# CEA-LIST/runia_core

Hardware: AMD Instinct MI355X
Metric: OOD scores/sec, LaREM 16-MC PCA-256 (ResNet-18 layer4 latent 512x4x4) (higher is better)
Workload: dtype f64

## Files before the change

### runia_core_amd/csrc/fused.hip

```cpp
#include "common.hpp"
#include "entropy_core.hpp"
#include "mfma_f64_tile.hpp"
#include "philox.hpp"
#include "div_consts.hpp"
#include "trap_order.hpp"

namespace {

using namespace runia_entropy;
using namespace runia_mfma;

constexpr int kMaxMC = 64;
typedef float f2 __attribute__((ext_vector_type(2)));

__device__ __forceinline__ void layer_consts(int cnt, int& m, float& flag, float& zh, float& zl) {
  const int a = cnt ? __ffs(cnt) - 1 : 0;
  m = cnt >> a;
  flag = __uint_as_float((unsigned)(127 - a) << 23);
  zh = cnt ? __uint_as_float(runia_div::kDivHi[(m - 1) >> 1]) : NAN;
  zl = cnt ? __uint_as_float(runia_div::kDivLo[(m - 1) >> 1]) : 0.f;
}

__device__ __forceinline__ float add_f32(float a, float b) {
  float r;
// ... 402 lines not shown
  const double* packed_ct;
  const double* bias;
  const double* scale;
  const double* md_mean;
  const double* packed_p;
  double* score;
  double* y_out;
  int64_t N, D, n;
};

template <int RT>
__global__ __launch_bounds__(256) void pca_md_kernel(PcaMdArgs g) {
  constexpr int BM = 16 * RT;
  extern __shared__ double lds[];
  const int64_t n_pad = n_padded(g.n);
  const int ypitch = (int)n_pad + 2;
  double* lds_a = lds;
  double* lds_y = lds + 2 * BM * APITCH;
  double* part = lds_y + (size_t)BM * ypitch;
  const int tid = threadIdx.x, lane = tid & 63;
  const int wave = __builtin_amdgcn_readfirstlane(tid >> 6);
  const int li = lane & 15, lg = lane >> 4;
  const int64_t NT = n_pad / 16;
  const int64_t r0 = (int64_t)blockIdx.x * BM;

  if (g.packed_ct) {
    const int64_t nchunks = k_padded(g.D) / KC;
    constexpr int PER_T = BM * KC / 256;
    for (int64_t cb = 0; cb < n_pad / BN; ++cb) {
      const int64_t ctbase = cb * 16 + wave * 4;
      d4 acc[RT][4];
#pragma unroll
      for (int a = 0; a < RT; ++a)
#pragma unroll
        for (int c = 0; c < 4; ++c) acc[a][c] = (d4){0.0, 0.0, 0.0, 0.0};
      const double2* bp = reinterpret_cast<const double2*>(g.packed_ct) + ctbase * 64 + lane;
      double2 b0[4];
#pragma unroll
      for (int c = 0; c < 4; ++c) b0[c] = bp[c * 64];
      double areg[PER_T];
      const int srow = (tid * PER_T) / KC, skk = (tid * PER_T) % KC;
      auto load_a = [&](int64_t kc) {
        const int64_t gr = r0 + srow;
#pragma unroll
        for (int q = 0; q < PER_T; ++q) {
          const int64_t gk = kc + skk + q;
          areg[q] = (gr < g.N && gk < g.D) ? g.h[gr * g.D + gk] : 0.0;
        }
      };
      load_a(0);
      int buf = 0;
      for (int64_t ch = 0; ch < nchunks; ++ch) {
#pragma unroll
        for (int q = 0; q < PER_T; ++q) lds_a[(buf * BM + srow) * APITCH + skk + q] = areg[q];
        __syncthreads();
        if (ch + 1 < nchunks) load_a((ch + 1) * KC);
        mfma_chunk<RT>(acc, lds_a + buf * BM * APITCH, APITCH, li, lg, bp + ch * 4 * NT * 64, NT * 64, b0);
        buf ^= 1;
      }
#pragma unroll
      for (int a = 0; a < RT; ++a)
#pragma unroll
        for (int c = 0; c < 4; ++c) {
          const int64_t col = (ctbase + c) * 16 + li;
#pragma unroll
          for (int r = 0; r < 4; ++r) {
            const int row = 16 * a + lg + 4 * r;
            double d = 0.0;
            if (col < g.n) {
              double y = acc[a][c][r] - g.bias[col];
              if (g.scale) y = y / g.scale[col];
              if (g.y_out && r0 + row < g.N) g.y_out[(r0 + row) * g.n + col] = y;
              d = y - g.md_mean[col];
            }
            lds_y[row * ypitch + col] = d;
          }
        }
      __syncthreads();
    }
  } else {
    for (int i = tid; i < BM * (int)n_pad; i += 256) {
      const int row = i / (int)n_pad, col = i - row * (int)n_pad;
      double d = 0.0;
      if (r0 + row < g.N && col < g.n) d = g.h[(r0 + row) * g.D + col] - g.md_mean[col];
      lds_y[row * ypitch + col] = d;
    }
    __syncthreads();
  }

  double rowdot[RT][4];
#pragma unroll
  for (int a = 0; a < RT; ++a)
#pragma unroll
    for (int r = 0; r < 4; ++r) rowdot[a][r] = 0.0;
  const int64_t kchunks = k_padded(g.n) / KC;
  for (int64_t cb = 0; cb < n_pad / BN; ++cb) {
    const int64_t ctbase = cb * 16 + wave * 4;
    d4 acc[RT][4];
#pragma unroll
    for (int a = 0; a < RT; ++a)
#pragma unroll
      for (int c = 0; c < 4; ++c) acc[a][c] = (d4){0.0, 0.0, 0.0, 0.0};
    const double2* bp = reinterpret_cast<const double2*>(g.packed_p) + ctbase * 64 + lane;
    double2 b0[4];
#pragma unroll
    for (int c = 0; c < 4; ++c) b0[c] = bp[c * 64];
    for (int64_t ch = 0; ch < kchunks; ++ch)
      mfma_chunk<RT>(acc, lds_y + ch * KC, ypitch, li, lg, bp + ch * 4 * NT * 64, NT * 64, b0);
#pragma unroll
    for (int a = 0; a < RT; ++a)
#pragma unroll
      for (int c = 0; c < 4; ++c) {
        const int col = (int)((ctbase + c) * 16) + li;
#pragma unroll
        for (int r = 0; r < 4; ++r) rowdot[a][r] += acc[a][c][r] * lds_y[(16 * a + lg + 4 * r) * ypitch + col];
      }
  }
#pragma unroll
  for (int a = 0; a < RT; ++a)
#pragma unroll
    for (int r = 0; r < 4; ++r) {
      double v = rowdot[a][r];
      v += shfl_xor_f64(v, 1);
      v += shfl_xor_f64(v, 2);
      v += shfl_xor_f64(v, 4);
      v += shfl_xor_f64(v, 8);
      if (li == 0) part[wave * BM + 16 * a + lg + 4 * r] = v;
    }
  __syncthreads();
  if (tid < BM) {
    const int64_t row = r0 + tid;
    if (row < g.N) g.score[row] = -(((part[tid] + part[BM + tid]) + part[2 * BM + tid]) + part[3 * BM + tid]);
  }
}

struct ProjSqArgs {
  const double* h;
  const double* packed_m;
  const double* c;
  double* score;
  double* partial;
  int64_t N, D, r;
};

#ifndef K2_WAVES
#define K2_WAVES 5
#endif
#ifndef K2_DMA
#define K2_DMA 1
#endif
#ifndef K2_WAVES_DMA
#define K2_WAVES_DMA 5
#endif
#ifndef K2_TRAP_FORM
#define K2_TRAP_FORM 2
#endif
#ifndef K2_TRAP_ROT
#define K2_TRAP_ROT 2
#endif
#ifndef K2_TRAP_HALFMAP
#define K2_TRAP_HALFMAP 1
#endif
template <int RT, int NCT, bool ACCUMULATE, bool SPLIT, bool DMA, int TRAP = 0>
__global__ __launch_bounds__(256, (RT == 1 && NCT <= 2) ? (DMA ? K2_WAVES_DMA : K2_WAVES) : 1) void proj_sq_kernel(ProjSqArgs g) {
#if defined(__HIP_DEVICE_COMPILE__)
  constexpr int BM = 16 * RT;
  constexpr bool WAVE_SKIP = TRAP >= 2 && DMA && RT == 1;
  __shared__ double lds_a[DMA ? 1 : 2 * BM * APITCH];
  __shared__ __attribute__((aligned(16))) double lds_d0[DMA ? BM * KC : 2];
  __shared__ __attribute__((aligned(16))) double lds_d1[DMA ? BM * KC : 2];
  constexpr int NG = (NCT + 1) / 2;
  __shared__ double part[4 * NG * BM];
  const int64_t n_pad = n_padded(g.r);
  const int tid = threadIdx.x, lane = tid & 63;
  const int wave = __builtin_amdgcn_readfirstlane(tid >> 6);
  const int li = lane & 15, lg = lane >> 4;
  const int64_t NT = n_pad / 16;
  int64_t tile = blockIdx.x;
  int half = 0;
  if constexpr (SPLIT) {
    tile = (int64_t)(blockIdx.x >> 4) * 8 + (blockIdx.x & 7);
    const unsigned j = blockIdx.x >> 3;
    half = (int)((K2_TRAP_HALFMAP ? j ^ (j >> 5) : j) & 1);
    if (tile * BM >= g.N) return;
  }
  const int64_t r0 = tile * BM;
  const int nchunks = (int)(k_padded(g.D) / KC);
  const int rot = K2_TRAP_ROT == 1 ? (int)(tile & 3)
                  : K2_TRAP_ROT == 2 ? (int)(((blockIdx.x >> 4) + (blockIdx.x >> 8)) & 3)
                  : K2_TRAP_ROT == 3 ? (int)((blockIdx.x >> 8) & 3) : 0;
  const int grp = WAVE_SKIP ? (wave + rot) & 3 : wave;
  constexpr int PER_T = BM * KC / 256;
  double rowsq[NG][RT][4];
#pragma unroll
  for (int q = 0; q < NG; ++q)
#pragma unroll
    for (int a = 0; a < RT; ++a)
#pragma unroll
      for (int r = 0; r < 4; ++r) rowsq[q][a][r] = 0.0;
  for (int64_t cb = 0; cb < n_pad / BN; ++cb) {
    const int64_t ctbase = cb * 16 + (int64_t)half * (4 * NCT) + grp * NCT;
    int64_t wg_chunk = (cb * 16 + (int64_t)half * (4 * NCT)) * 16 / KC, wave_chunk = ctbase * 16 / KC;
    if constexpr (TRAP == 3) {
      const int64_t wg_pos = (cb * 16 + (int64_t)half * (4 * NCT)) / 2, wave_pos = ctbase / 2;
      wg_chunk = trap_balanced_first_k(wg_pos, g.r) / KC;
#pragma unroll
      for (int i = 1; i < 2 * NCT; ++i) {
        const int64_t f = trap_balanced_first_k(wg_pos + i, g.r) / KC;
        wg_chunk = f < wg_chunk ? f : wg_chunk;
      }
      wave_chunk = trap_balanced_first_k(wave_pos, g.r) / KC;
#pragma unroll
      for (int q = 1; q < NG; ++q) {
        const int64_t f = trap_balanced_first_k(wave_pos + q, g.r) / KC;
        wave_chunk = f < wave_chunk ? f : wave_chunk;
      }
    }
    const int ch0 = TRAP ? (int)(wg_chunk < nchunks - 1 ? wg_chunk : nchunks - 1) : 0;
    [[maybe_unused]] const int ws = WAVE_SKIP ? (int)(wave_chunk < nchunks - 1 ? wave_chunk : nchunks - 1) : ch0;
    d4 acc[RT][NCT];
#pragma unroll
    for (int a = 0; a < RT; ++a)
#pragma unroll
      for (int c = 0; c < NCT; ++c) acc[a][c] = (d4){0.0, 0.0, 0.0, 0.0};
    double2 bring[4][NCT];
    if constexpr (DMA) {
      const __amdgpu_buffer_rsrc_t brsrc = buffer_of(g.packed_m, (unsigned)(packed_elems(g.D, g.r) * 8));
      const int64_t rows_here = (g.N - r0 < BM) ? g.N - r0 : BM;
      const __amdgpu_buffer_rsrc_t arsrc = buffer_of(g.h + r0 * g.D, (unsigned)(rows_here * g.D * 8));
      const unsigned lane_bytes = (unsigned)lane * 16u;
      const unsigned pair_stride_bytes = (unsigned)NT * 1024u;
      const unsigned ct_bytes = (unsigned)ctbase * 1024u;
      constexpr int NDMA = BM / 4 / 4;
      unsigned a_lane_bytes[NDMA];
#pragma unroll
      for (int i = 0; i < NDMA; ++i) {
        const int slot = 64 * (wave + 4 * i) + lane;
        a_lane_bytes[i] = (unsigned)(((slot % BM) * g.D + 2 * (slot / BM)) * 8);
      }
      auto dma_rows = [&](int bufc, int kc) {
#pragma unroll
        for (int i = 0; i < NDMA; ++i)
          __builtin_amdgcn_raw_ptr_buffer_load_lds(
              arsrc, (__attribute__((address_space(3))) void*)((bufc ? lds_d1 : lds_d0) + 128 * (wave + 4 * i)), 16,
              a_lane_bytes[i], (unsigned)kc * 8u, 0, 0);
        asm volatile("" ::: "memory");
      };
      auto body = [&](auto buf_tag, int ch) {
        constexpr int bufc = decltype(buf_tag)::value;
        asm volatile("s_waitcnt vmcnt(%0)" ::"n"(3 * NCT) : "memory");
        __syncthreads();
        dma_rows(bufc ^ 1, ((ch + 1 < nchunks) ? ch + 1 : ch) * KC);
        mfma_chunk_dma<RT, NCT, BM>(acc, bufc ? lds_d1 : lds_d0, li, lg, brsrc, lane_bytes,
                                    ct_bytes + (unsigned)ch * 4u * pair_stride_bytes, pair_stride_bytes, bring);
      };
      dma_rows(0, ch0 * KC);
      int ch = ch0;
      if constexpr (WAVE_SKIP) {
        for (; ch < ws; ++ch) {
          asm volatile("s_waitcnt vmcnt(0)" ::: "memory");
          __syncthreads();
          dma_rows((ch + 1 - ch0) & 1, (ch + 1) * KC);
        }
      }
#pragma unroll
      for (int j = 0; j < 3; ++j)
#pragma unroll
        for (int c = 0; c < NCT; ++c)
          bring[j][c] = __builtin_bit_cast(double2, __builtin_amdgcn_raw_buffer_load_b128(
                                                        brsrc, lane_bytes + c * 1024u,
                                                        ct_bytes + (unsigned)(4 * ch + j) * pair_stride_bytes, 0));
      if constexpr (WAVE_SKIP) {
        if ((ch - ch0) & 1) {
          body(std::integral_constant<int, 1>{}, ch);
          ++ch;
        }
      }
      for (; ch + 1 < nchunks; ch += 2) {
        body(std::integral_constant<int, 0>{}, ch);
        body(std::integral_constant<int, 1>{}, ch + 1);
      }
      if (ch < nchunks) body(std::integral_constant<int, 0>{}, ch);
    } else {
      const double2* bp = reinterpret_cast<const double2*>(g.packed_m) + ctbase * 64 + lane + (int64_t)ch0 * 4 * NT * 64;
    #pragma unroll
      for (int j = 0; j < 3; ++j)
  #pragma unroll
        for (int c = 0; c < NCT; ++c) bring[j][c] = bp[j * NT * 64 + c * 64];
      double areg[PER_T];
      const int srow = tid / KC, skk = tid % KC;
      const bool interior = (r0 + BM <= g.N) && (g.D % KC == 0);
      const double* pa = g.h + (r0 + srow) * g.D + skk;
      auto load_a = [&](int64_t kc) {
        if (interior) {
  #pragma unroll
          for (int q = 0; q < PER_T; ++q) areg[q] = pa[(int64_t)q * (256 / KC) * g.D + kc];
          return;
        }
        const int64_t gk = kc + skk;
  #pragma unroll
        for (int q = 0; q < PER_T; ++q) {
          const int64_t gr = r0 + srow + q * (256 / KC);
          areg[q] = (gr < g.N && gk < g.D) ? g.h[gr * g.D + gk] : 0.0;
        }
      };
      load_a((int64_t)ch0 * KC);
      int buf = 0;
      for (int64_t ch = ch0; ch < nchunks; ++ch) {
  #pragma unroll
        for (int q = 0; q < PER_T; ++q) lds_a[(buf * BM + srow + q * (256 / KC)) * APITCH + skk] = areg[q];
        __syncthreads();
        if (ch + 1 < nchunks) load_a((ch + 1) * KC);
        mfma_chunk_ring<RT, NCT>(acc, lds_a + buf * BM * APITCH, APITCH, li, lg, bp + (ch - ch0) * 4 * NT * 64, NT * 64, bring);
        buf ^= 1;
      }
    }
#pragma unroll
    for (int a = 0; a < RT; ++a)
#pragma unroll
      for (int c = 0; c < NCT; ++c) {
        const int64_t col = (ctbase + c) * 16 + li;
        const double cc = (col < g.r) ? g.c[col] : 0.0;
#pragma unroll
        for (int r = 0; r < 4; ++r) {
          const double v = acc[a][c][r] + cc;
          rowsq[c / 2][a][r] = fma(v, v, rowsq[c / 2][a][r]);
        }
      }
    __syncthreads();
  }
#pragma unroll
  for (int q = 0; q < NG; ++q)
#pragma unroll
    for (int a = 0; a < RT; ++a)
#pragma unroll
      for (int r = 0; r < 4; ++r) {
        double v = rowsq[q][a][r];
        v += shfl_xor_f64(v, 1);
        v += shfl_xor_f64(v, 2);
        v += shfl_xor_f64(v, 4);
        v += shfl_xor_f64(v, 8);
        if (li == 0) part[(grp * NG + q) * BM + 16 * a + lg + 4 * r] = v;
      }
  __syncthreads();
  if (tid < BM) {
    const int64_t row = r0 + tid;
    if (row < g.N) {
      const double lo = ((part[tid] + part[BM + tid]) + part[2 * BM + tid]) + part[3 * BM + tid];
      if constexpr (NCT == 4) {
        const double hi = ((part[4 * BM + tid] + part[5 * BM + tid]) + part[6 * BM + tid]) + part[7 * BM + tid];
        g.score[row] = -(lo + hi);
      } else if constexpr (!SPLIT) {
        if constexpr (ACCUMULATE) unsafeAtomicAdd(&g.score[row], -lo);
        else g.score[row] = -lo;
      } else if constexpr (ACCUMULATE) {
        unsafeAtomicAdd(&g.score[row], -lo);
      } else {
        g.partial[(int64_t)half * g.N + row] = lo;
      }
    }
  }
#endif
}

__global__ void proj_sq_combine_kernel(const double* __restrict__ partial, double* __restrict__ score, int64_t N) {
  const int64_t i = (int64_t)blockIdx.x * blockDim.x + threadIdx.x;
  if (i < N) score[i] = -(partial[i] + partial[N + i]);
}

double digamma_diff(int n, int k) {
  double s = 0.0;
  for (int j = n - 1; j >= k; --j) s += 1.0 / (double)j;
  return s;
}

template <int RT>
int launch_pca_md(const PcaMdArgs& g, hipStream_t s) {
  constexpr int BM = 16 * RT;
  const int64_t n_pad = n_padded(g.n);
  const size_t shmem = ((size_t)2 * BM * APITCH + (size_t)BM * (n_pad + 2) + 4 * BM) * sizeof(double);
  if (shmem > 160 * 1024) return RUNIA_E_INVALID;
  static std::atomic<uint64_t> lds_ok{0};
  if (runia_allow_dynamic_lds(reinterpret_cast<const void*>(pca_md_kernel<RT>), 160 * 1024, lds_ok) != RUNIA_OK)
    return RUNIA_E_LAUNCH;
  const int64_t tiles = (g.N + BM - 1) / BM;
  pca_md_kernel<RT><<<(unsigned)tiles, 256, shmem, s>>>(g);
  return runia_check_launch();
}

}

extern "C" int runia_pca_md_score_f64(const double* h, const double* packed_ct, const double* bias,
                                      const double* scale, const double* md_mean, const double* packed_p,
                                      double* score, double* y_out, int64_t N, int64_t D, int64_t n,
                                      runia_stream_t stream) {
  if (N < 0 || D <= 0 || n <= 0) return RUNIA_E_INVALID;
  if (N == 0) return RUNIA_OK;
  if (!h || !md_mean || !packed_p || !score) return RUNIA_E_INVALID;
  if (packed_ct ? !bias : (n != D)) return RUNIA_E_INVALID;
  PcaMdArgs g{h, packed_ct, bias, scale, md_mean, packed_p, score, y_out, N, D, n};
  const int64_t tiles32 = (N + 31) / 32;
  const int64_t n_pad = n_padded(n);
  const bool fits32 = ((size_t)2 * 32 * APITCH + (size_t)32 * (n_pad + 2) + 128) * 8 <= 160 * 1024;
  if (tiles32 >= 1024 && fits32) return launch_pca_md<2>(g, as_stream(stream));
  return launch_pca_md<1>(g, as_stream(stream));
}

namespace {
template <int HH, int WW, int NPP>
void launch_mask(const float* rnd, int64_t rand_image_stride, float* table, int64_t N, int n_mc, float gamma,
                 int block_size, int identity, int sort_layers, uint64_t seed, int64_t first_image, int redraw,
                 hipStream_t s) {
  static_assert(HH * WW <= 64, "mc_mask_bits_kernel holds a drop layer in one 64-bit word");
  const unsigned grid = (unsigned)((N + kMaskBitsWaves - 1) / kMaskBitsWaves);
  if (redraw)
    mc_mask_bits_kernel<HH, WW, NPP, true><<<grid, 64 * kMaskBitsWaves, 0, s>>>(rnd, rand_image_stride, table, N, n_mc, gamma,
                                                                              block_size, identity, sort_layers, seed, first_image);
  else
    mc_mask_bits_kernel<HH, WW, NPP, false><<<grid, 64 * kMaskBitsWaves, 0, s>>>(rnd, rand_image_stride, table, N, n_mc, gamma,
                                                                               block_size, identity, sort_layers, seed, first_image);
}

__global__ void mc_draws_kernel(float* __restrict__ out, int64_t N, int per_image, uint64_t seed, int64_t first_image) {
  const int64_t i = (int64_t)blockIdx.x * blockDim.x + threadIdx.x;
  if (i >= N * per_image) return;
  const int64_t img = i / per_image;
  out[i] = runia_philox::draw(seed, (uint64_t)(first_image + img), (int)(i - img * per_image));
}
}

extern "C" int runia_mc_entropy_supported(int H, int W, int n_mc, int k);

extern "C" size_t runia_mc_entropy_workspace_bytes(int64_t N, int H, int W, int n_mc) {
  if (N <= 0 || H <= 0 || W <= 0 || n_mc <= 0) return 0;
  return (size_t)N * (size_t)n_mc * (size_t)(H * W + 2) * sizeof(float);
}

static int mc_args_ok(int64_t N, int H, int W, int n_mc, const void* workspace, size_t workspace_bytes) {
  if (N < 0 || N > 65535 || H <= 0 || W <= 0 || n_mc < 2 || n_mc > kMaxMC) return RUNIA_E_INVALID;
  if (N == 0) return RUNIA_OK;
  if (!workspace || workspace_bytes < runia_mc_entropy_workspace_bytes(N, H, W, n_mc) ||
      (((uintptr_t)workspace) & 15) != 0)
    return RUNIA_E_WORKSPACE;
  return RUNIA_OK;
}

#define RUNIA_MCE_SHAPES(F) \
  F(4, 4, 16, 5) F(4, 4, 32, 5) F(4, 4, 8, 5) F(2, 2, 16, 5) F(2, 2, 32, 5) F(7, 7, 16, 5) F(7, 7, 32, 5) F(8, 8, 16, 5) F(8, 8, 32, 5)

static int mc_mask_table(const float* rnd, int64_t rand_image_stride, void* workspace, size_t workspace_bytes,
                         int64_t N, int H, int W, int n_mc, double drop_prob, int block_size, int sort_layers,
                         runia_stream_t stream, bool counter = false, uint64_t seed = 0, int64_t first_image = 0,
                         int redraw = 0) {
  if (block_size < 1) return RUNIA_E_INVALID;
  if (int rc = mc_args_ok(N, H, W, n_mc, workspace, workspace_bytes)) return rc;
  if (N == 0) return RUNIA_OK;
  const int identity = (drop_prob == 0.0);
  if (!identity && !rnd && !counter) return RUNIA_E_INVALID;
  if (counter) rnd = nullptr;
  float* table = reinterpret_cast<float*>(workspace);
  const float gamma = (float)(drop_prob / (double)(block_size * block_size));
  hipStream_t s = as_stream(stream);
#define RUNIA_MCE(HH, WW, NPP, KK)                                                                          \
  if (H == HH && W == WW && n_mc <= NPP && n_mc > NPP / 2) {                                                \
    launch_mask<HH, WW, NPP>(rnd, rand_image_stride, table, N, n_mc, gamma, block_size, identity,           \
                             sort_layers, seed, first_image, redraw, s);                                    \
    return runia_check_launch();                                                                            \
  }
  RUNIA_MCE_SHAPES(RUNIA_MCE)
#undef RUNIA_MCE
  return RUNIA_E_INVALID;
}

extern "C" int runia_mc_mask_table_f32(const float* rnd, int64_t rand_image_stride, void* workspace,
                                       size_t workspace_bytes, int64_t N, int H, int W, int n_mc, double drop_prob,
                                       int block_size, runia_stream_t stream) {
  return mc_mask_table(rnd, rand_image_stride, workspace, workspace_bytes, N, H, W, n_mc, drop_prob, block_size, 1,
                       stream);
}

extern "C" int runia_mc_stack_table_f32(const float* x, const float* rnd, int64_t rand_image_stride, float* z,
                                        void* workspace, size_t workspace_bytes, int64_t N, int C, int H, int W,
                                        int n_mc, double drop_prob, int block_size, runia_stream_t stream) {
  if (C <= 0) return RUNIA_E_INVALID;
  if (int rc = mc_args_ok(N, H, W, n_mc, workspace, workspace_bytes)) return rc;
  if (N == 0) return RUNIA_OK;
  if (!x || !z || !runia_mc_entropy_supported(H, W, n_mc, 5)) return RUNIA_E_INVALID;
  if (!(((((uintptr_t)x) & 15) == 0) || (H * W) % 4 != 0)) return RUNIA_E_INVALID;
  if (int rc = mc_mask_table(rnd, rand_image_stride, workspace, workspace_bytes, N, H, W, n_mc, drop_prob,
                             block_size, 0, stream))
    return rc;
  const float* table = reinterpret_cast<const float*>(workspace);
  const unsigned grid = (unsigned)((((N + 7) / 8 + K1_IMGS - 1) / K1_IMGS) * 8 * ((C + kK1Block - 1) / kK1Block));
  hipStream_t s = as_stream(stream);
#define RUNIA_MCE(HH, WW, NPP, KK)                                                                          \
// ... 27 lines not shown
  const unsigned grid = (unsigned)((((N + 7) / 8 + K1_IMGS - 1) / K1_IMGS) * 8 * ((C + kK1Block - 1) / kK1Block));
  hipStream_t s = as_stream(stream);
  const bool x16 = ((((uintptr_t)x) & 15) == 0);
#define RUNIA_MCE(HH, WW, NPP, KK)                                                                          \
  if (H == HH && W == WW && n_mc <= NPP && n_mc > NPP / 2 && k == KK && (x16 || (HH * WW) % 4 != 0)) {      \
    if (n_mc == NPP)                                                                                        \
      RUNIA_LAUNCH_TIMED((mc_entropy_kernel<HH, WW, NPP, KK, true>), grid, kK1Block, 0, s, x, table, h, z_out, \
                         zero_fill, N, C, n_mc, min_dist, ct, inv_n);                                       \
    else                                                                                                    \
      RUNIA_LAUNCH_TIMED((mc_entropy_kernel<HH, WW, NPP, KK, false>), grid, kK1Block, 0, s, x, table, h, z_out, \
                         zero_fill, N, C, n_mc, min_dist, ct, inv_n);                                       \
    return runia_check_launch();                                                                            \
  }
  RUNIA_MCE_SHAPES(RUNIA_MCE)
#undef RUNIA_MCE
  return RUNIA_E_INVALID;
}

extern "C" int runia_mc_entropy_f32(const float* x, const float* rnd, int64_t rand_image_stride, double* h,
                                    float* z_out, double* zero_fill, void* workspace, size_t workspace_bytes,
                                    int64_t N, int C, int H, int W, int n_mc, double drop_prob, int block_size,
                                    int k, double min_dist, runia_stream_t stream) {
  if (N < 0 || C <= 0 || H <= 0 || W <= 0 || n_mc < 2 || n_mc > kMaxMC || block_size < 1 || k < 1 || k >= n_mc)
    return RUNIA_E_INVALID;
  if (N == 0) return RUNIA_OK;
  if (!x || !h || N > 65535) return RUNIA_E_INVALID;
  if (!runia_mc_entropy_supported(H, W, n_mc, k)) return RUNIA_E_INVALID;
  if (drop_prob != 0.0 && !rnd) return RUNIA_E_INVALID;
  if (!(((((uintptr_t)x) & 15) == 0) || (H * W) % 4 != 0)) return RUNIA_E_INVALID;
  if (int rc = runia_mc_mask_table_f32(rnd, rand_image_stride, workspace, workspace_bytes, N, H, W, n_mc, drop_prob,
                                       block_size, stream))
    return rc;
  return runia_mc_entropy_from_table_f32(x, workspace, workspace_bytes, h, z_out, zero_fill, N, C, H, W, n_mc, k,
                                         min_dist, stream);
}

int runia_roi_sample_table(const float* feat_nhwc, const float* boxes, const int* batch_idx, void* table, size_t table_bytes,
                           int64_t K, int64_t B, int C, int H, int W, int PH, int PW, double spatial_scale, int G, int aligned,
                           hipStream_t s);
size_t runia_roi_sample_table_bytes(int64_t K, int PH, int PW, int G);

#define RUNIA_ROI_MCE_SHAPES(X)                                                                                    \
  X(7, 7, 16, 5, 2) X(7, 7, 32, 5, 2) X(7, 7, 16, 5, 1) X(7, 7, 32, 5, 1)                                          \
  X(4, 4, 16, 5, 2) X(4, 4, 32, 5, 2) X(8, 8, 16, 5, 2) X(8, 8, 32, 5, 2)

extern "C" int runia_roi_mc_entropy_supported(int PH, int PW, int n_mc, int k, int sampling_ratio) {
  if (!runia_mc_entropy_supported(PH, PW, n_mc, k)) return 0;
#define RUNIA_ROI_HAS(HH, WW, NPP, KK, GG) \
  if (PH == HH && PW == WW && n_mc <= NPP && n_mc > NPP / 2 && k == KK && sampling_ratio == GG) return 1;
  RUNIA_ROI_MCE_SHAPES(RUNIA_ROI_HAS)
#undef RUNIA_ROI_HAS
  return 0;
}
extern "C" size_t runia_roi_mc_entropy_workspace_bytes(int64_t K, int PH, int PW, int n_mc, int sampling_ratio) {
  if (K <= 0 || sampling_ratio < 1) return 0;
  const size_t masks = (runia_mc_entropy_workspace_bytes(K, PH, PW, n_mc) + 255) / 256 * 256;
  return masks + runia_roi_sample_table_bytes(K, PH, PW, sampling_ratio);
}
extern "C" int runia_roi_mc_entropy_f32(const float* feat_nhwc, const float* boxes, const int* batch_idx, const float* rnd,
                                        int64_t rand_image_stride, double* h, float* z_out, void* workspace,
                                        size_t workspace_bytes, int64_t K, int64_t B, int C, int H, int W, int PH, int PW,
                                        double spatial_scale, int sampling_ratio, int aligned, int n_mc, double drop_prob,
                                        int block_size, int k, double min_dist, runia_stream_t stream) {
  if (K < 0 || B <= 0 || C <= 0 || H <= 0 || W <= 0 || n_mc < 2 || n_mc > kMaxMC || block_size < 1 || k < 1 || k >= n_mc)
    return RUNIA_E_INVALID;
  if (K == 0) return RUNIA_OK;
  if (!feat_nhwc || !boxes || !h || K > 65535 || (B > 1 && !batch_idx)) return RUNIA_E_INVALID;
  if (!runia_roi_mc_entropy_supported(PH, PW, n_mc, k, sampling_ratio)) return RUNIA_E_INVALID;
  if ((int64_t)H * W * C * 4 >= ((int64_t)1 << 30)) return RUNIA_E_INVALID;
  if (drop_prob != 0.0 && !rnd) return RUNIA_E_INVALID;
  if (!workspace || (((uintptr_t)workspace) & 15) != 0 ||
      workspace_bytes < runia_roi_mc_entropy_workspace_bytes(K, PH, PW, n_mc, sampling_ratio))
    return RUNIA_E_WORKSPACE;
  const size_t masks = (runia_mc_entropy_workspace_bytes(K, PH, PW, n_mc) + 255) / 256 * 256;
  if (int rc = runia_mc_mask_table_f32(rnd, rand_image_stride, workspace, masks, K, PH, PW, n_mc, drop_prob, block_size, stream))
    return rc;
  char* tab = reinterpret_cast<char*>(workspace) + masks;
  hipStream_t s = as_stream(stream);
  if (int rc = runia_roi_sample_table(feat_nhwc, boxes, batch_idx, tab, workspace_bytes - masks, K, B, C, H, W, PH, PW,
                                      spatial_scale, sampling_ratio, aligned, s))
    return rc;
  const float* table = reinterpret_cast<const float*>(workspace);
  const float* src = reinterpret_cast<const float*>(tab);
  const double ct = digamma_diff(n_mc, k), inv_n = 1.0 / (double)n_mc;
  const unsigned grid = (unsigned)((((K + 7) / 8 + K1_IMGS - 1) / K1_IMGS) * 8 * ((C + kK1Block - 1) / kK1Block));
#define RUNIA_ROI_MCE(HH, WW, NPP, KK, GG)                                                                         \
  if (PH == HH && PW == WW && n_mc <= NPP && n_mc > NPP / 2 && k == KK && sampling_ratio == GG) {                  \
    if (n_mc == NPP)                                                                                               \
      mc_entropy_kernel<HH, WW, NPP, KK, true, true, GG><<<grid, kK1Block, 0, s>>>(src, table, h, z_out, nullptr,  \
                                                                                   K, C, n_mc, min_dist, ct, inv_n); \
    else                                                                                                           \
      mc_entropy_kernel<HH, WW, NPP, KK, false, true, GG><<<grid, kK1Block, 0, s>>>(src, table, h, z_out, nullptr, \
                                                                                    K, C, n_mc, min_dist, ct, inv_n); \
    return runia_check_launch();                                                                                   \
  }
  RUNIA_ROI_MCE_SHAPES(RUNIA_ROI_MCE)
#undef RUNIA_ROI_MCE
  return RUNIA_E_INVALID;
}

extern "C" int runia_mc_draws_f32(float* out, int64_t N, int n_mc, int H, int W, uint64_t seed, int64_t first_image,
                                  runia_stream_t stream) {
  if (N < 0 || n_mc < 1 || H <= 0 || W <= 0 || first_image < 0 || (int64_t)n_mc * H * W > (1 << 20))
    return RUNIA_E_INVALID;
  if (N == 0) return RUNIA_OK;
  if (!out) return RUNIA_E_INVALID;
  const int64_t total = N * n_mc * H * W;
  if ((total + 255) / 256 > 0x7fffffffLL) return RUNIA_E_INVALID;
  mc_draws_kernel<<<(unsigned)((total + 255) / 256), 256, 0, as_stream(stream)>>>(out, N, n_mc * H * W, seed,
                                                                                first_image);
  return runia_check_launch();
}

extern "C" int runia_mc_mask_table_counter_f32(uint64_t seed, int64_t first_image, void* workspace,
                                               size_t workspace_bytes, int64_t N, int H, int W, int n_mc,
                                               double drop_prob, int block_size, int redraw_dead_layers,
                                               runia_stream_t stream) {
  if (first_image < 0) return RUNIA_E_INVALID;
  return mc_mask_table(nullptr, 0, workspace, workspace_bytes, N, H, W, n_mc, drop_prob, block_size, 1, stream, true,
                       seed, first_image, redraw_dead_layers ? 1 : 0);
}

extern "C" int runia_mc_entropy_counter_f32(const float* x, uint64_t seed, int64_t first_image, double* h,
                                            float* z_out, double* zero_fill, void* workspace, size_t workspace_bytes,
                                            int64_t N, int C, int H, int W, int n_mc, double drop_prob,
                                            int block_size, int k, double min_dist, int redraw_dead_layers,
                                            runia_stream_t stream) {
  if (N < 0 || C <= 0 || H <= 0 || W <= 0 || n_mc < 2 || n_mc > kMaxMC || block_size < 1 || k < 1 || k >= n_mc ||
      first_image < 0)
    return RUNIA_E_INVALID;
  if (N == 0) return RUNIA_OK;
  if (!x || !h || N > 65535) return RUNIA_E_INVALID;
  if (!runia_mc_entropy_supported(H, W, n_mc, k)) return RUNIA_E_INVALID;
  if (!(((((uintptr_t)x) & 15) == 0) || (H * W) % 4 != 0)) return RUNIA_E_INVALID;
  if (int rc = runia_mc_mask_table_counter_f32(seed, first_image, workspace, workspace_bytes, N, H, W, n_mc,
                                               drop_prob, block_size, redraw_dead_layers, stream))
    return rc;
  return runia_mc_entropy_from_table_f32(x, workspace, workspace_bytes, h, z_out, zero_fill, N, C, H, W, n_mc, k,
                                         min_dist, stream);
}

extern "C" int runia_mc_entropy_supported(int H, int W, int n_mc, int k) {
  if (k != 5 || k >= n_mc) return 0;
  const bool hw = (H == 4 && W == 4);
  if (hw && n_mc > 4 && n_mc <= 32) return 1;
  if (n_mc > 8 && n_mc <= 32 && ((H == 2 && W == 2) || (H == 7 && W == 7) || (H == 8 && W == 8))) return 1;
  return 0;
}

static bool proj_sq_dma_ok(int64_t D, int64_t r) {
  return K2_DMA && D % KC == 0 && D < (1 << 23) && packed_elems(D, r) < ((int64_t)1 << 29);
}
static bool proj_sq_one_round(unsigned grid) { return (int64_t)grid <= (int64_t)K2_WAVES_DMA * runia_cu_count(); }
template <int TRAP, int RT, int NCT, bool ACCUMULATE, bool SPLIT>
static void launch_proj_sq(unsigned grid, hipStream_t s, const ProjSqArgs& g, bool dma) {
  const bool use_dma = dma && (RT > 1 || proj_sq_one_round(grid));
  if constexpr (TRAP) {
    constexpr int FORM = TRAP == 2 ? 3 : K2_TRAP_FORM;
    if (use_dma) proj_sq_kernel<RT, NCT, ACCUMULATE, SPLIT, true, FORM><<<grid, 256, 0, s>>>(g);
    else if constexpr (RT > 1) proj_sq_kernel<RT, NCT, ACCUMULATE, SPLIT, false, FORM><<<grid, 256, 0, s>>>(g);
    else proj_sq_kernel<RT, NCT, ACCUMULATE, SPLIT, false><<<grid, 256, 0, s>>>(g);
  } else {
    if (use_dma) proj_sq_kernel<RT, NCT, ACCUMULATE, SPLIT, true><<<grid, 256, 0, s>>>(g);
    else proj_sq_kernel<RT, NCT, ACCUMULATE, SPLIT, false><<<grid, 256, 0, s>>>(g);
  }
}

static bool proj_sq_large_tiles(int64_t N, int64_t cus) {
  const int64_t tiles32 = (N + 31) / 32;
  const int64_t rounds = (tiles32 + cus - 1) / cus;
  return tiles32 >= 2 * cus && 100 * tiles32 >= 93 * rounds * cus;
}

template <int TRAP>
static int proj_sq_accumulate(const double* h, const double* packed_m, const double* c, double* score, int64_t N, int64_t D,
                              int64_t r, runia_stream_t stream) {
  if (N < 0 || D <= 0 || r <= 0) return RUNIA_E_INVALID;
  if (N == 0) return RUNIA_OK;
  if (!h || !packed_m || !c || !score) return RUNIA_E_INVALID;
  ProjSqArgs g{h, packed_m, c, score, nullptr, N, D, r};
  hipStream_t s = as_stream(stream);
  const int64_t tiles16 = (N + 15) / 16, cus = runia_cu_count();
  const bool dma = proj_sq_dma_ok(D, r);
  if (r <= 64) launch_proj_sq<TRAP, 1, 1, true, false>((unsigned)tiles16, s, g, dma);
  else if (r <= 128) launch_proj_sq<TRAP, 1, 2, true, false>((unsigned)tiles16, s, g, dma);
  else if (proj_sq_large_tiles(N, cus)) launch_proj_sq<TRAP, 2, 4, false, false>((unsigned)((N + 31) / 32), s, g, dma);
  else if (tiles16 > cus / 2) launch_proj_sq<TRAP, 1, 2, true, true>((unsigned)((tiles16 + 7) / 8 * 16), s, g, dma);
  else launch_proj_sq<TRAP, 1, 4, false, false>((unsigned)tiles16, s, g, dma);
  return runia_check_launch();
}

extern "C" int runia_proj_sq_accumulate_f64(const double* h, const double* packed_m, const double* c, double* score,
                                            int64_t N, int64_t D, int64_t r, runia_stream_t stream) {
  return proj_sq_accumulate<0>(h, packed_m, c, score, N, D, r, stream);
}
extern "C" int runia_proj_sq_accumulate_trap_f64(const double* h, const double* packed_m, const double* c, double* score,
                                                 int64_t N, int64_t D, int64_t r, runia_stream_t stream) {
  if (r > D) return RUNIA_E_INVALID;
  return proj_sq_accumulate<1>(h, packed_m, c, score, N, D, r, stream);
}
extern "C" int runia_proj_sq_accumulate_btrap_f64(const double* h, const double* packed_m, const double* c, double* score,
                                                  int64_t N, int64_t D, int64_t r, runia_stream_t stream) {
  if (r > D) return RUNIA_E_INVALID;
  return proj_sq_accumulate<2>(h, packed_m, c, score, N, D, r, stream);
}

extern "C" size_t runia_proj_sq_workspace_bytes(int64_t N) { return N > 0 ? (size_t)N * 2 * sizeof(double) : 0; }

template <int TRAP>
static int proj_sq_score(const double* h, const double* packed_m, const double* c, double* score, void* workspace,
                         size_t workspace_bytes, int64_t N, int64_t D, int64_t r, runia_stream_t stream) {
  if (N < 0 || D <= 0 || r <= 0) return RUNIA_E_INVALID;
  if (N == 0) return RUNIA_OK;
  if (!h || !packed_m || !c || !score) return RUNIA_E_INVALID;
  ProjSqArgs g{h, packed_m, c, score, reinterpret_cast<double*>(workspace), N, D, r};
  hipStream_t s = as_stream(stream);
  const int64_t tiles16 = (N + 15) / 16, cus = runia_cu_count();
  const bool dma = proj_sq_dma_ok(D, r);
  if (r <= 64) {
    launch_proj_sq<TRAP, 1, 1, false, false>((unsigned)tiles16, s, g, dma);
  } else if (r <= 128) {
    launch_proj_sq<TRAP, 1, 2, false, false>((unsigned)tiles16, s, g, dma);
  } else if (proj_sq_large_tiles(N, cus)) {
    launch_proj_sq<TRAP, 2, 4, false, false>((unsigned)((N + 31) / 32), s, g, dma);
  } else if (tiles16 > cus / 2 && workspace && workspace_bytes >= runia_proj_sq_workspace_bytes(N)) {
    launch_proj_sq<TRAP, 1, 2, false, true>((unsigned)((tiles16 + 7) / 8 * 16), s, g, dma);
    proj_sq_combine_kernel<<<(unsigned)((N + 255) / 256), 256, 0, s>>>(g.partial, score, N);
  } else {
    launch_proj_sq<TRAP, 1, 4, false, false>((unsigned)tiles16, s, g, dma);
  }
  return runia_check_launch();
}

extern "C" int runia_proj_sq_score_f64(const double* h, const double* packed_m, const double* c, double* score,
                                       void* workspace, size_t workspace_bytes, int64_t N, int64_t D, int64_t r,
                                       runia_stream_t stream) {
  return proj_sq_score<0>(h, packed_m, c, score, workspace, workspace_bytes, N, D, r, stream);
}
extern "C" int runia_proj_sq_score_trap_f64(const double* h, const double* packed_m, const double* c, double* score,
                                            void* workspace, size_t workspace_bytes, int64_t N, int64_t D, int64_t r,
                                            runia_stream_t stream) {
  if (r > D) return RUNIA_E_INVALID;
  return proj_sq_score<1>(h, packed_m, c, score, workspace, workspace_bytes, N, D, r, stream);
}
extern "C" int runia_proj_sq_score_btrap_f64(const double* h, const double* packed_m, const double* c, double* score,
                                             void* workspace, size_t workspace_bytes, int64_t N, int64_t D, int64_t r,
                                             runia_stream_t stream) {
  if (r > D) return RUNIA_E_INVALID;
  return proj_sq_score<2>(h, packed_m, c, score, workspace, workspace_bytes, N, D, r, stream);
}
```

### runia_core_amd/csrc/mfma_f64_tile.hpp

```cpp
#pragma once
#include "common.hpp"

namespace runia_mfma {

constexpr int KC = 32;
constexpr int APITCH = 34;
constexpr int BN = 256;

__host__ __device__ inline int64_t n_padded(int64_t n) { return (n + BN - 1) / BN * BN; }
__host__ __device__ inline int64_t k_padded(int64_t K) { return (K + KC - 1) / KC * KC; }
__host__ __device__ inline int64_t packed_pairs(int64_t K) { return k_padded(K) / 8 + 4; }
__host__ __device__ inline int64_t packed_elems(int64_t K, int64_t n) { return packed_pairs(K) * 8 * n_padded(n); }

template <int RT, int NCT = 4>
__device__ __forceinline__ void mfma_chunk(d4 (&acc)[RT][NCT], const double* a_tile, int pitch, int li, int lg,
                                           const double2* __restrict__ bp, int64_t pair_stride,
                                           double2 (&b0)[NCT]) {
  double av[RT][8];
#pragma unroll
  for (int a = 0; a < RT; ++a)
#pragma unroll
    for (int t = 0; t < 8; ++t) av[a][t] = a_tile[(16 * a + li) * pitch + 4 * t + lg];
  double2 b1[NCT];
#pragma unroll
  for (int s2 = 0; s2 < 4; ++s2) {
    if ((s2 & 1) == 0) {
#pragma unroll
      for (int c = 0; c < NCT; ++c) b1[c] = bp[(s2 + 1) * pair_stride + c * 64];
    } else {
#pragma unroll
      for (int c = 0; c < NCT; ++c) b0[c] = bp[(s2 + 1) * pair_stride + c * 64];
    }
#pragma unroll
    for (int hh = 0; hh < 2; ++hh) {
#pragma unroll
      for (int c = 0; c < NCT; ++c) {
        const double2 bb = (s2 & 1) ? b1[c] : b0[c];
        const double bv = hh ? bb.y : bb.x;
#pragma unroll
        for (int a = 0; a < RT; ++a)
          acc[a][c] = __builtin_amdgcn_mfma_f64_16x16x4f64(av[a][2 * s2 + hh], bv, acc[a][c], 0, 0, 0);
      }
    }
  }
}

template <int RT, int NCT>
__device__ __forceinline__ void mfma_chunk_ring(d4 (&acc)[RT][NCT], const double* a_tile, int pitch, int li, int lg,
                                                const double2* __restrict__ bp, int64_t pair_stride,
                                                double2 (&b)[4][NCT]) {
  double av[RT][8];
#pragma unroll
  for (int a = 0; a < RT; ++a)
#pragma unroll
    for (int t = 0; t < 8; ++t) av[a][t] = a_tile[(16 * a + li) * pitch + 4 * t + lg];
#pragma unroll
  for (int s2 = 0; s2 < 4; ++s2) {
#pragma unroll
    for (int c = 0; c < NCT; ++c) b[(s2 + 3) & 3][c] = bp[(s2 + 3) * pair_stride + c * 64];
#pragma unroll
    for (int hh = 0; hh < 2; ++hh) {
#pragma unroll
      for (int c = 0; c < NCT; ++c) {
        const double bv = hh ? b[s2][c].y : b[s2][c].x;
#pragma unroll
        for (int a = 0; a < RT; ++a)
          acc[a][c] = __builtin_amdgcn_mfma_f64_16x16x4f64(av[a][2 * s2 + hh], bv, acc[a][c], 0, 0, 0);
      }
    }
  }
}

#if defined(__HIP_DEVICE_COMPILE__)
using u4 = unsigned __attribute__((ext_vector_type(4)));
__device__ __forceinline__ __amdgpu_buffer_rsrc_t buffer_of(const void* base, unsigned bytes) {
  return __builtin_amdgcn_make_buffer_rsrc(const_cast<void*>(base), 0, (int)bytes, 0x00020000);
}

template <int RT, int NCT, int BM>
__device__ __forceinline__ void mfma_chunk_dma(d4 (&acc)[RT][NCT], const double* a_slots, int li, int lg,
                                               __amdgpu_buffer_rsrc_t brsrc, unsigned lane_bytes, unsigned pair0_bytes,
                                               unsigned pair_stride_bytes, double2 (&b)[4][NCT]) {
  double av[RT][8];
#pragma unroll
  for (int a = 0; a < RT; ++a)
#pragma unroll
    for (int t = 0; t < 8; ++t) av[a][t] = a_slots[(((2 * t + (lg >> 1)) * BM + 16 * a + li) << 1) + (lg & 1)];
#pragma unroll
  for (int s2 = 0; s2 < 4; ++s2) {
#pragma unroll
    for (int c = 0; c < NCT; ++c) {
      const u4 v = __builtin_amdgcn_raw_buffer_load_b128(brsrc, lane_bytes + c * 1024u,
                                                         pair0_bytes + (unsigned)(s2 + 3) * pair_stride_bytes, 0);
      b[(s2 + 3) & 3][c] = __builtin_bit_cast(double2, v);
    }
#pragma unroll
    for (int hh = 0; hh < 2; ++hh) {
#pragma unroll
      for (int c = 0; c < NCT; ++c) {
        const double bv = hh ? b[s2][c].y : b[s2][c].x;
#pragma unroll
        for (int a = 0; a < RT; ++a)
          acc[a][c] = __builtin_amdgcn_mfma_f64_16x16x4f64(av[a][2 * s2 + hh], bv, acc[a][c], 0, 0, 0);
      }
    }
  }
}
#endif

}
```

### runia_core_amd/csrc/trap_order.hpp

```cpp
#pragma once
#include <cstdint>

__host__ __device__ inline int64_t trap_balanced_block(int64_t pos, int64_t r) {
  const int64_t cb = pos >> 3;
  if ((cb + 1) * 256 > r) return pos;
  return cb * 8 + ((0x74216530u >> (4 * (unsigned)(pos & 7))) & 7u);
}

__host__ __device__ inline int64_t trap_balanced_first_k(int64_t pos, int64_t r) { return 32 * trap_balanced_block(pos, r); }
```

Baseline: 61.63 million.

## Add 64-k DMA step variant for projection-square kernel with half-step trapezoid entry

```diff
diff --git a/runia_core_amd/csrc/fused.hip b/runia_core_amd/csrc/fused.hip
--- a/runia_core_amd/csrc/fused.hip
+++ b/runia_core_amd/csrc/fused.hip
@@ -578,23 +578,24 @@
 #ifndef K2_WAVES_DMA
 #define K2_WAVES_DMA 5
 #endif
+#ifndef K2_DMA_KC
+#define K2_DMA_KC 64
+#endif
+static_assert(K2_DMA_KC == 32 || K2_DMA_KC == 64, "32 or 64 k per DMA step");
 #ifndef K2_TRAP_FORM
 #define K2_TRAP_FORM 2
-#endif
-#ifndef K2_TRAP_ROT
-#define K2_TRAP_ROT 2
 #endif
 #ifndef K2_TRAP_HALFMAP
 #define K2_TRAP_HALFMAP 1
 #endif
-template <int RT, int NCT, bool ACCUMULATE, bool SPLIT, bool DMA, int TRAP = 0>
+template <int RT, int NCT, bool ACCUMULATE, bool SPLIT, bool DMA, int TRAP = 0, int KCD = KC>
 __global__ __launch_bounds__(256, (RT == 1 && NCT <= 2) ? (DMA ? K2_WAVES_DMA : K2_WAVES) : 1) void proj_sq_kernel(ProjSqArgs g) {
 #if defined(__HIP_DEVICE_COMPILE__)
   constexpr int BM = 16 * RT;
   constexpr bool WAVE_SKIP = TRAP >= 2 && DMA && RT == 1;
   __shared__ double lds_a[DMA ? 1 : 2 * BM * APITCH];
-  __shared__ __attribute__((aligned(16))) double lds_d0[DMA ? BM * KC : 2];
-  __shared__ __attribute__((aligned(16))) double lds_d1[DMA ? BM * KC : 2];
+  __shared__ __attribute__((aligned(16))) double lds_d0[DMA ? BM * KCD : 2];
+  __shared__ __attribute__((aligned(16))) double lds_d1[DMA ? BM * KCD : 2];
   constexpr int NG = (NCT + 1) / 2;
   __shared__ double part[4 * NG * BM];
   const int64_t n_pad = n_padded(g.r);
@@ -612,10 +613,7 @@
   }
   const int64_t r0 = tile * BM;
   const int nchunks = (int)(k_padded(g.D) / KC);
-  const int rot = K2_TRAP_ROT == 1 ? (int)(tile & 3)
-                  : K2_TRAP_ROT == 2 ? (int)(((blockIdx.x >> 4) + (blockIdx.x >> 8)) & 3)
-                  : K2_TRAP_ROT == 3 ? (int)((blockIdx.x >> 8) & 3) : 0;
-  const int grp = WAVE_SKIP ? (wave + rot) & 3 : wave;
+  const int grp = wave;
   constexpr int PER_T = BM * KC / 256;
   double rowsq[NG][RT][4];
 #pragma unroll
@@ -626,19 +624,20 @@
       for (int r = 0; r < 4; ++r) rowsq[q][a][r] = 0.0;
   for (int64_t cb = 0; cb < n_pad / BN; ++cb) {
     const int64_t ctbase = cb * 16 + (int64_t)half * (4 * NCT) + grp * NCT;
-    int64_t wg_chunk = (cb * 16 + (int64_t)half * (4 * NCT)) * 16 / KC, wave_chunk = ctbase * 16 / KC;
+    using chunk_t = std::conditional_t<KCD == KC, int64_t, int>;
+    chunk_t wg_chunk = (chunk_t)((cb * 16 + (int64_t)half * (4 * NCT)) * 16 / KC), wave_chunk = (chunk_t)(ctbase * 16 / KC);
     if constexpr (TRAP == 3) {
       const int64_t wg_pos = (cb * 16 + (int64_t)half * (4 * NCT)) / 2, wave_pos = ctbase / 2;
-      wg_chunk = trap_balanced_first_k(wg_pos, g.r) / KC;
+      wg_chunk = (chunk_t)(trap_balanced_first_k((chunk_t)wg_pos, (chunk_t)g.r) / KC);
 #pragma unroll
       for (int i = 1; i < 2 * NCT; ++i) {
-        const int64_t f = trap_balanced_first_k(wg_pos + i, g.r) / KC;
+        const chunk_t f = (chunk_t)(trap_balanced_first_k((chunk_t)(wg_pos + i), (chunk_t)g.r) / KC);
         wg_chunk = f < wg_chunk ? f : wg_chunk;
       }
-      wave_chunk = trap_balanced_first_k(wave_pos, g.r) / KC;
+      wave_chunk = (chunk_t)(trap_balanced_first_k((chunk_t)wave_pos, (chunk_t)g.r) / KC);
 #pragma unroll
       for (int q = 1; q < NG; ++q) {
-        const int64_t f = trap_balanced_first_k(wave_pos + q, g.r) / KC;
+        const chunk_t f = (chunk_t)(trap_balanced_first_k((chunk_t)(wave_pos + q), (chunk_t)g.r) / KC);
         wave_chunk = f < wave_chunk ? f : wave_chunk;
       }
     }
@@ -657,7 +656,7 @@
       const unsigned lane_bytes = (unsigned)lane * 16u;
       const unsigned pair_stride_bytes = (unsigned)NT * 1024u;
       const unsigned ct_bytes = (unsigned)ctbase * 1024u;
-      constexpr int NDMA = BM / 4 / 4;
+      constexpr int NDMA = BM * KCD / 512;
       unsigned a_lane_bytes[NDMA];
 #pragma unroll
       for (int i = 0; i < NDMA; ++i) {
@@ -672,41 +671,92 @@
               a_lane_bytes[i], (unsigned)kc * 8u, 0, 0);
         asm volatile("" ::: "memory");
       };
-      auto body = [&](auto buf_tag, int ch) {
-        constexpr int bufc = decltype(buf_tag)::value;
-        asm volatile("s_waitcnt vmcnt(%0)" ::"n"(3 * NCT) : "memory");
-        __syncthreads();
-        dma_rows(bufc ^ 1, ((ch + 1 < nchunks) ? ch + 1 : ch) * KC);
-        mfma_chunk_dma<RT, NCT, BM>(acc, bufc ? lds_d1 : lds_d0, li, lg, brsrc, lane_bytes,
-                                    ct_bytes + (unsigned)ch * 4u * pair_stride_bytes, pair_stride_bytes, bring);
-      };
-      dma_rows(0, ch0 * KC);
-      int ch = ch0;
-      if constexpr (WAVE_SKIP) {
-        for (; ch < ws; ++ch) {
-          asm volatile("s_waitcnt vmcnt(0)" ::: "memory");
+      if constexpr (KCD == KC) {
+        auto body = [&](auto buf_tag, int ch) {
+          constexpr int bufc = decltype(buf_tag)::value;
+          asm volatile("s_waitcnt vmcnt(%0)" ::"n"(3 * NCT) : "memory");
           __syncthreads();
-          dma_rows((ch + 1 - ch0) & 1, (ch + 1) * KC);
-        }
-      }
-#pragma unroll
-      for (int j = 0; j < 3; ++j)
-#pragma unroll
-        for (int c = 0; c < NCT; ++c)
-          bring[j][c] = __builtin_bit_cast(double2, __builtin_amdgcn_raw_buffer_load_b128(
-                                                        brsrc, lane_bytes + c * 1024u,
-                                                        ct_bytes + (unsigned)(4 * ch + j) * pair_stride_bytes, 0));
-      if constexpr (WAVE_SKIP) {
-        if ((ch - ch0) & 1) {
-          body(std::integral_constant<int, 1>{}, ch);
-          ++ch;
-        }
-      }
-      for (; ch + 1 < nchunks; ch += 2) {
-        body(std::integral_constant<int, 0>{}, ch);
-        body(std::integral_constant<int, 1>{}, ch + 1);
-      }
-      if (ch < nchunks) body(std::integral_constant<int, 0>{}, ch);
+          dma_rows(bufc ^ 1, ((ch + 1 < nchunks) ? ch + 1 : ch) * KC);
+          mfma_chunk_dma<RT, NCT, BM>(acc, bufc ? lds_d1 : lds_d0, li, lg, brsrc, lane_bytes,
+                                      ct_bytes + (unsigned)ch * 4u * pair_stride_bytes, pair_stride_bytes, bring);
+        };
+        dma_rows(0, ch0 * KC);
+        int ch = ch0;
+        if constexpr (WAVE_SKIP) {
+          for (; ch < ws; ++ch) {
+            asm volatile("s_waitcnt vmcnt(0)" ::: "memory");
+            __syncthreads();
+            dma_rows((ch + 1 - ch0) & 1, (ch + 1) * KC);
+          }
+        }
+  #pragma unroll
+        for (int j = 0; j < 3; ++j)
+  #pragma unroll
+          for (int c = 0; c < NCT; ++c)
+            bring[j][c] = __builtin_bit_cast(double2, __builtin_amdgcn_raw_buffer_load_b128(
+                                                          brsrc, lane_bytes + c * 1024u,
+                                                          ct_bytes + (unsigned)(4 * ch + j) * pair_stride_bytes, 0));
+        if constexpr (WAVE_SKIP) {
+          if ((ch - ch0) & 1) {
+            body(std::integral_constant<int, 1>{}, ch);
+            ++ch;
+          }
+        }
+        for (; ch + 1 < nchunks; ch += 2) {
+          body(std::integral_constant<int, 0>{}, ch);
+          body(std::integral_constant<int, 1>{}, ch + 1);
+        }
+        if (ch < nchunks) body(std::integral_constant<int, 0>{}, ch);
+      } else {
+        static_assert(KCD == 2 * KC, "a 64-k step is two 32-k halves");
+        const int n64 = nchunks / 2;
+        const int c0 = ch0 >> 1;
+        auto step = [&](auto buf_tag, int ch, auto first_half_tag) {
+          constexpr int bufc = decltype(buf_tag)::value;
+          asm volatile("s_waitcnt vmcnt(%0)" ::"n"(3 * NCT) : "memory");
+          __syncthreads();
+          dma_rows(bufc ^ 1, ((ch + 1 < n64) ? ch + 1 : ch) * KCD);
+          mfma_step64_dma<RT, NCT, BM, decltype(first_half_tag)::value>(acc, bufc ? lds_d1 : lds_d0, li, lg, brsrc, lane_bytes,
+                                                                        ct_bytes + (unsigned)ch * 8u * pair_stride_bytes,
+                                                                        pair_stride_bytes, bring);
+        };
+        auto body = [&](auto buf_tag, int ch) { step(buf_tag, ch, std::true_type{}); };
+        auto half_body = [&](auto buf_tag, int ch) { step(buf_tag, ch, std::false_type{}); };
+        dma_rows(0, c0 * KCD);
+        int ch = c0;
+        if constexpr (WAVE_SKIP) {
+          for (; ch < (ws >> 1); ++ch) {
+            asm volatile("s_waitcnt vmcnt(0)" ::: "memory");
+            __syncthreads();
+            dma_rows((ch + 1 - c0) & 1, (ch + 1) * KCD);
+          }
+        }
+#pragma unroll
+        for (int j = 0; j < 3; ++j)
+#pragma unroll
+          for (int c = 0; c < NCT; ++c)
+            bring[j][c] = __builtin_bit_cast(double2, __builtin_amdgcn_raw_buffer_load_b128(
+                                                          brsrc, lane_bytes + c * 1024u,
+                                                          ct_bytes + (unsigned)(4 * ws + j) * pair_stride_bytes, 0));
+        if constexpr (TRAP != 0) {
+          if (ws & 1) {
+            if ((ch - c0) & 1) half_body(std::integral_constant<int, 1>{}, ch);
+            else half_body(std::integral_constant<int, 0>{}, ch);
+            ++ch;
+          }
+        }
+        if constexpr (TRAP != 0) {
+          if (((ch - c0) & 1) && ch < n64) {
+            body(std::integral_constant<int, 1>{}, ch);
+            ++ch;
+          }
+        }
+        for (; ch + 1 < n64; ch += 2) {
+          body(std::integral_constant<int, 0>{}, ch);
+          body(std::integral_constant<int, 1>{}, ch + 1);
+        }
+        if (ch < n64) body(std::integral_constant<int, 0>{}, ch);
+      }
     } else {
       const double2* bp = reinterpret_cast<const double2*>(g.packed_m) + ctbase * 64 + lane + (int64_t)ch0 * 4 * NT * 64;
     #pragma unroll
@@ -746,7 +796,15 @@
 #pragma unroll
       for (int c = 0; c < NCT; ++c) {
         const int64_t col = (ctbase + c) * 16 + li;
-        const double cc = (col < g.r) ? g.c[col] : 0.0;
+        double cc;
+        if constexpr (DMA && KCD != KC) {
+          using u2 = unsigned __attribute__((ext_vector_type(2)));
+          const u2 v = __builtin_amdgcn_raw_buffer_load_b64(buffer_of(g.c, (unsigned)(g.r * 8)), (unsigned)li * 8u,
+                                                            (unsigned)(ctbase + c) * 128u, 0);
+          cc = __builtin_bit_cast(double, v);
+        } else {
+          cc = (col < g.r) ? g.c[col] : 0.0;
+        }
 #pragma unroll
         for (int r = 0; r < 4; ++r) {
           const double v = acc[a][c][r] + cc;
@@ -755,6 +813,9 @@
       }
     __syncthreads();
   }
+  int etid = tid;
+  if constexpr (DMA && KCD != KC) asm volatile("" : "+v"(etid));
+  const int eli = etid & 15, elg = (etid & 63) >> 4;
 #pragma unroll
   for (int q = 0; q < NG; ++q)
 #pragma unroll
@@ -766,7 +827,7 @@
         v += shfl_xor_f64(v, 2);
         v += shfl_xor_f64(v, 4);
         v += shfl_xor_f64(v, 8);
-        if (li == 0) part[(grp * NG + q) * BM + 16 * a + lg + 4 * r] = v;
+        if (eli == 0) part[(grp * NG + q) * BM + 16 * a + elg + 4 * r] = v;
       }
   __syncthreads();
   if (tid < BM) {
@@ -1100,11 +1161,22 @@
   return K2_DMA && D % KC == 0 && D < (1 << 23) && packed_elems(D, r) < ((int64_t)1 << 29);
 }
 static bool proj_sq_one_round(unsigned grid) { return (int64_t)grid <= (int64_t)K2_WAVES_DMA * runia_cu_count(); }
+template <int TRAP, int RT, int NCT, bool SPLIT>
+static constexpr bool proj_sq_form_has_kc64() { return K2_DMA_KC == 64 && RT == 1 && NCT > 1 && !(SPLIT && TRAP != 0); }
+static bool proj_sq_kc64(bool split, unsigned grid, int64_t D) {
+  return D % (2 * KC) == 0 && (split || (int64_t)grid <= runia_cu_count() / 2);
+}
 template <int TRAP, int RT, int NCT, bool ACCUMULATE, bool SPLIT>
 static void launch_proj_sq(unsigned grid, hipStream_t s, const ProjSqArgs& g, bool dma) {
   const bool use_dma = dma && (RT > 1 || proj_sq_one_round(grid));
+  constexpr int FORM = TRAP == 0 ? 0 : TRAP == 2 ? 3 : K2_TRAP_FORM;
+  if constexpr (proj_sq_form_has_kc64<TRAP, RT, NCT, SPLIT>()) {
+    if (use_dma && proj_sq_kc64(SPLIT, grid, g.D)) {
+      proj_sq_kernel<RT, NCT, ACCUMULATE, SPLIT, true, FORM, 2 * KC><<<grid, 256, 0, s>>>(g);
+      return;
+    }
+  }
   if constexpr (TRAP) {
-    constexpr int FORM = TRAP == 2 ? 3 : K2_TRAP_FORM;
     if (use_dma) proj_sq_kernel<RT, NCT, ACCUMULATE, SPLIT, true, FORM><<<grid, 256, 0, s>>>(g);
     else if constexpr (RT > 1) proj_sq_kernel<RT, NCT, ACCUMULATE, SPLIT, false, FORM><<<grid, 256, 0, s>>>(g);
     else proj_sq_kernel<RT, NCT, ACCUMULATE, SPLIT, false><<<grid, 256, 0, s>>>(g);
diff --git a/runia_core_amd/csrc/mfma_f64_tile.hpp b/runia_core_amd/csrc/mfma_f64_tile.hpp
--- a/runia_core_amd/csrc/mfma_f64_tile.hpp
+++ b/runia_core_amd/csrc/mfma_f64_tile.hpp
@@ -106,6 +106,40 @@
     }
   }
 }
+
+template <int RT, int NCT, int BM, bool FIRST>
+__device__ __forceinline__ void mfma_step64_dma(d4 (&acc)[RT][NCT], const double* a_slots, int li, int lg,
+                                                __amdgpu_buffer_rsrc_t brsrc, unsigned lane_bytes, unsigned pair0_bytes,
+                                                unsigned pair_stride_bytes, double2 (&b)[4][NCT]) {
+  double av[2][RT][8];
+  auto read_a = [&](int h) {
+#pragma unroll
+    for (int a = 0; a < RT; ++a)
+#pragma unroll
+      for (int t = 0; t < 8; ++t) av[h][a][t] = a_slots[(((16 * h + 2 * t + (lg >> 1)) * BM + 16 * a + li) << 1) + (lg & 1)];
+  };
+  read_a(FIRST ? 0 : 1);
+#pragma unroll
+  for (int s2 = FIRST ? 0 : 4; s2 < 8; ++s2) {
+#pragma unroll
+    for (int c = 0; c < NCT; ++c) {
+      const u4 v = __builtin_amdgcn_raw_buffer_load_b128(brsrc, lane_bytes + c * 1024u,
+                                                         pair0_bytes + (unsigned)(s2 + 3) * pair_stride_bytes, 0);
+      b[(s2 + 3) & 3][c] = __builtin_bit_cast(double2, v);
+    }
+#pragma unroll
+    for (int hh = 0; hh < 2; ++hh) {
+#pragma unroll
+      for (int c = 0; c < NCT; ++c) {
+        const double bv = hh ? b[s2 & 3][c].y : b[s2 & 3][c].x;
+#pragma unroll
+        for (int a = 0; a < RT; ++a)
+          acc[a][c] = __builtin_amdgcn_mfma_f64_16x16x4f64(av[s2 >> 2][a][2 * (s2 & 3) + hh], bv, acc[a][c], 0, 0, 0);
+      }
+    }
+    if (FIRST && s2 == 2) read_a(1);
+  }
+}
 #endif
 
 }
diff --git a/runia_core_amd/csrc/trap_order.hpp b/runia_core_amd/csrc/trap_order.hpp
--- a/runia_core_amd/csrc/trap_order.hpp
+++ b/runia_core_amd/csrc/trap_order.hpp
@@ -1,10 +1,12 @@
 #pragma once
 #include <cstdint>
 
-__host__ __device__ inline int64_t trap_balanced_block(int64_t pos, int64_t r) {
-  const int64_t cb = pos >> 3;
+template <class I>
+__host__ __device__ inline I trap_balanced_block(I pos, I r) {
+  const I cb = pos >> 3;
   if ((cb + 1) * 256 > r) return pos;
-  return cb * 8 + ((0x74216530u >> (4 * (unsigned)(pos & 7))) & 7u);
+  return cb * 8 + (I)((0x74216530u >> (4 * (unsigned)(pos & 7))) & 7u);
 }
 
-__host__ __device__ inline int64_t trap_balanced_first_k(int64_t pos, int64_t r) { return 32 * trap_balanced_block(pos, r); }
+template <class I>
+__host__ __device__ inline I trap_balanced_first_k(I pos, I r) { return 32 * trap_balanced_block(pos, r); }
```

New measurement: 59.63 million. 3.2% lower.
